# YiyangShao/splendor-gym

Measured on AMD Instinct MI355X. Metric: env-steps/sec (whole node), 2p 65536 tables/GPU, higher is better.
Workload: dtype int32

## Files before the change

### include/splendor_amd.h

```cpp
#ifndef SPLENDOR_AMD_H
#define SPLENDOR_AMD_H

#include <stdint.h>

#include "splendor_table.h"

#ifdef __cplusplus
extern "C" {
#endif

#define SPL_ABI_VERSION 9

#define SPL_F_ILLEGAL 0x01
#define SPL_F_DRAW 0x02
#define SPL_F_TURN_LIMIT 0x04
#define SPL_F_AFTER_TERMINAL 0x08
#define SPL_F_OOB 0x10
#define SPL_F_RESET 0x20
#define SPL_F_RNG_LIMIT 0x40
#define SPL_F_FAULT 0x80

#define SPL_POLICY_UNIFORM 0
#define SPL_POLICY_GREEDY_V1 1
#define SPL_POLICY_BASIC_PRIORITY 2
// ... 26 lines not shown
    int32_t autoreset;
    int32_t policy;
    int32_t *next_actions;
    const uint64_t *ply_base;
    uint64_t policy_seed;
    uint64_t ply;
    int64_t table0;
    float *ep_return;
    uint32_t *ep_count;
    uint8_t *info;
    uint64_t *errors;
    uint8_t *obs_u8;
    const uint8_t *gate_terminated;
    const uint8_t *gate_flags;
} spl_step_args_t;

int spl_abi_version(void);
const char *spl_last_error(void);

int spl_ctx_create(int device, const int32_t *cards, const int32_t *nobles, spl_ctx_t **out);
int spl_ctx_destroy(spl_ctx_t *ctx);
int spl_ctx_set_refill_period(spl_ctx_t *ctx, int period);
int spl_ctx_set_refill_fused(spl_ctx_t *ctx, int fused);
int spl_ctx_set_rollout_pipeline(spl_ctx_t *ctx, int on);
int spl_ctx_set_rollout_delegation(spl_ctx_t *ctx, int every);
int spl_ctx_set_partner_lead(spl_ctx_t *ctx, int lead);
int spl_ctx_set_step_tail(spl_ctx_t *ctx, int mode);
const char *spl_rollout_kernel_name(spl_ctx_t *ctx, int32_t n, int32_t players, int32_t per_step_outputs);

int spl_ctx_faults(spl_ctx_t *ctx, uint64_t *launch, int clear);
const volatile uint64_t *spl_ctx_fault_word(spl_ctx_t *ctx);
uint64_t spl_ctx_launches(spl_ctx_t *ctx);
int spl_host_mapped(const void *host, int32_t *same_address);

int64_t spl_arena_bytes(int32_t n, int32_t players);
int spl_arena_init(spl_ctx_t *ctx, spl_arena_t *arena, void *stream);

int spl_reset(spl_ctx_t *ctx, spl_arena_t *arena, const uint64_t *pcg, const uint8_t *reset_mask,
              int32_t *obs, int8_t *mask, void *stream);

int spl_deal(spl_ctx_t *ctx, spl_arena_t *arena, const uint32_t *engine_seeds, const uint8_t *deal_mask,
             int32_t *obs, int8_t *mask, void *stream);

int spl_step(spl_ctx_t *ctx, spl_arena_t *arena, const spl_step_args_t *args, void *stream);

int spl_rollout(spl_ctx_t *ctx, spl_arena_t *arena, const spl_step_args_t *args, int32_t steps,
                int32_t per_step_outputs, void *stream);

int spl_refill(spl_ctx_t *ctx, spl_arena_t *arena, void *stream);

int spl_encode(spl_ctx_t *ctx, spl_arena_t *arena, int32_t *obs, void *stream);
int spl_legal(spl_ctx_t *ctx, spl_arena_t *arena, int8_t *mask, void *stream);

int spl_sample_uniform(spl_ctx_t *ctx, int32_t n, const int8_t *mask, int32_t *actions,
                       uint64_t seed, uint64_t ply, int64_t table0, void *stream);

int spl_step_info(int32_t n, const uint8_t *flags, uint8_t *info, uint64_t *errors, void *stream);

int spl_table_download(spl_ctx_t *ctx, spl_arena_t *arena, int32_t first, int32_t count,
                       spl_table_t *host, void *stream);
int spl_table_upload(spl_ctx_t *ctx, spl_arena_t *arena, int32_t first, int32_t count,
                     const spl_table_t *host, void *stream);

int spl_debug_set_stream_limit(int outputs);

int spl_debug_set_spin_limit(int64_t polls);
int spl_debug_partner_stats(uint64_t *stats, int clear);

int spl_debug_bounds_flags(uint32_t *flags, int clear);

int64_t spl_ctx_token_lut(spl_ctx_t *ctx, uint32_t *out, int64_t words);

#ifdef __cplusplus
}
#endif
#endif
```

### splendor-gym_amd/csrc/spl_engine.hip

```cpp
#include <hip/hip_runtime.h>
#include <stdint.h>
#include <string.h>

#include <algorithm>
#include <atomic>
#include <map>
#include <mutex>
#include <string>
#include <vector>

#include "../../include/splendor_amd.h"
#include "spl_layout.h"
#include "spl_rng.h"

namespace spl {

struct KArena {
    uint32_t *planes;
    uint32_t *pool;
    uint8_t *slots;
    uint8_t *pcg;
    int n;
    uint8_t *deleg;
    uint32_t *dflags;
// ... 2979 lines not shown
        wave_lds_sync();
        if (obs) store_obs_block(L.rows, rows, obs + (size_t)t0 * kObsDim);
        if (mask_out) store_mask_block(L.mask, L.mbits, rows, mask_out + (size_t)t0 * 45);
    }
    if (valid) store_tab(T, A, t, lm, Tb.mtag);
}

constexpr int kRefillLds = 40 * 1024;
template <int P>
__global__ __launch_bounds__(64) void k_refill(KArena A) {
    __shared__ uint8_t scr_all[kRefillLds] __attribute__((aligned(16)));
    const int t = blockIdx.x * 64 + lane_id();
    if (t >= A.n) return;
    const size_t mi = (size_t)SW_MISC * A.n + t;
    const uint32_t misc = A.planes[mi];
    if (pend_of(misc) == 0) return;
    Deal pool;
    bool pool_dirty = false;
    A.planes[mi] = refill_table<P>(A, t, misc, &scr_all[lane_id() * kScratchStride],
                                   reinterpret_cast<uint32_t *>(&scr_all[64 * kScratchStride]), pool, pool_dirty);
    if (pool_dirty) store_pool(A, t, pool);
}

template <int P>
__global__ __launch_bounds__(64) void k_observe(KArena A, KTables Tb, int32_t *obs, int8_t *mask_out) {
    __shared__ BlockLDS L;
    const int lane = lane_id();
    const int t0 = blockIdx.x * 64;
    const int t = t0 + lane;
    const bool valid = t < A.n;
    const int rows = min(64, A.n - t0);
    load_tables_lds(L, Tb);
    Tab<P> T;
    if (valid) load_tab(T, A, t);
    else fresh_state(T, 0u, empty_deal());
    wave_lds_sync();
    if (obs) encode_row(T, L.rows, L);
    L.mask[lane] = valid ? legal_of(T, L) : 0ull;
    wave_lds_sync();
    if (obs) {
        store_obs_block(L.rows, rows, obs + (size_t)t0 * kObsDim);
        if (__any(valid && get_moves(T.sw) > 255)) {
            __builtin_amdgcn_s_waitcnt(0);
            if (valid && get_moves(T.sw) > 255) obs[(size_t)t * kObsDim + 295] = get_moves(T.sw);
        }
    }
// ... 168 lines not shown
}

using namespace spl;

struct spl_ctx_s {
    int device;
    uint4 *cards;
    uint2 *nobles;
    uint4 *lut;
    int refill_period;
    int refill_fused;
    int pipeline;
    int resident[7][5];
    int deleg_every;
    int partner_lead;
    uint32_t mtag;
    int step_tail;
    int64_t step_tail_blocks;
    uint64_t *fault_host;
    uint64_t *fault_dev;
    uint64_t launches;
    void *stage;
    size_t stage_bytes;
};

static thread_local std::string g_err;

int spl_fail(int code, const std::string &msg) {
    g_err = msg;
    return code;
}
static inline int fail(int code, const std::string &msg) { return spl_fail(code, msg); }

#define HIP_TRY(expr)                                                                   \
    do {                                                                                \
        hipError_t e_ = (expr);                                                         \
        if (e_ != hipSuccess) return fail(SPL_E_HIP, std::string(#expr ": ") + hipGetErrorString(e_)); \
    } while (0)

static KTables ktables(const spl_ctx_t *c) { return KTables{c->cards, c->nobles, c->lut, c->mtag}; }

static int check_arena(const spl_ctx_t *ctx, const spl_arena_t *a) {
    if (!ctx) return fail(SPL_E_ARG, "null context");
    if (!a || !a->base) return fail(SPL_E_ARG, "null arena");
    if (a->players < 2 || a->players > 4) return fail(SPL_E_ARG, "players must be 2..4");
    if (a->n <= 0) return fail(SPL_E_ARG, "arena must hold at least one table");
    if (((uintptr_t)a->base & 255u) != 0) return fail(SPL_E_ARG, "arena base must be 256-byte aligned");
    if (a->bytes < spl_arena_bytes(a->n, a->players)) return fail(SPL_E_ARG, "arena too small");
    return SPL_OK;
}

static KArena karena(const spl_arena_t *a) {
    const ArenaLayout L = arena_layout(a->n, a->players);
    uint8_t *b = static_cast<uint8_t *>(a->base);
    return KArena{reinterpret_cast<uint32_t *>(b + L.planes), reinterpret_cast<uint32_t *>(b + L.pool), b + L.slots,
                  b + L.pcg, a->n, b + L.deleg, reinterpret_cast<uint32_t *>(b + L.dflags),
                  reinterpret_cast<uint32_t *>(b + L.legal)};
}

static int launch_check() {
    hipError_t e = hipGetLastError();
    if (e != hipSuccess) return fail(SPL_E_HIP, std::string("kernel launch: ") + hipGetErrorString(e));
    return SPL_OK;
}

static inline unsigned blocks_for(int64_t n) { return (unsigned)((n + 63) / 64); }

extern "C" {

int spl_abi_version(void) { return SPL_ABI_VERSION; }

// ... 108 lines not shown
        memcpy(&nrec[i], b, 8);
    }
    HIP_TRY(hipSetDevice(device));
    int resident[7][5] = {};
    {
        int cus = 0;
        HIP_TRY(hipDeviceGetAttribute(&cus, hipDeviceAttributeMultiprocessorCount, device));
        for (int shape = 2; shape <= 6; ++shape)
            for (int p = 2; p <= 4; ++p) {
                const RolloutKernel &k = rollout_kernel(shape, true, p);
                int occ = 0;
                HIP_TRY(hipOccupancyMaxActiveBlocksPerMultiprocessor(&occ, k.fn, k.threads, 0));
                resident[shape][p] = occ * cus;
            }
    }
    spl_ctx_t *c = new spl_ctx_t();
    c->device = device;
    c->mtag = card_table_tag(crec, nrec);
    c->refill_period = 64;
    c->refill_fused = 1;
    c->deleg_every = kDelegEveryDefault;
    c->partner_lead = kPartnerLeadDefault;
    c->step_tail = -1;
    {
        int cus = 0;
        HIP_TRY(hipDeviceGetAttribute(&cus, hipDeviceAttributeMultiprocessorCount, device));
        c->step_tail_blocks = 3 * (int64_t)cus;
    }
    c->pipeline = 1;
    memcpy(c->resident, resident, sizeof(resident));
    if (hipMalloc(&c->cards, sizeof(uint4) * 90) != hipSuccess || hipMalloc(&c->nobles, sizeof(uint2) * 10) != hipSuccess ||
        hipMalloc(&c->lut, sizeof(uint4) * kLutEntries) != hipSuccess) {
        spl_ctx_destroy(c);
        return fail(SPL_E_HIP, "hipMalloc of constant tables failed");
    }
    if (hipHostMalloc(reinterpret_cast<void **>(&c->fault_host), sizeof(uint64_t),
                      hipHostMallocMapped | hipHostMallocCoherent) != hipSuccess ||
        hipHostGetDevicePointer(reinterpret_cast<void **>(&c->fault_dev), c->fault_host, 0) != hipSuccess) {
        spl_ctx_destroy(c);
        return fail(SPL_E_HIP, "hipHostMalloc of the fault word failed");
    }
    *c->fault_host = 0;
    HIP_TRY(hipMemcpy(c->cards, crec.data(), sizeof(uint4) * 90, hipMemcpyHostToDevice));
    HIP_TRY(hipMemcpy(c->nobles, nrec.data(), sizeof(uint2) * 10, hipMemcpyHostToDevice));
    hipLaunchKernelGGL(k_build_lut, dim3(blocks_for(kLutEntries)), dim3(64), 0, 0, c->lut);
    if (int r = launch_check()) {
        spl_ctx_destroy(c);
        return r;
    }
    HIP_TRY(hipDeviceSynchronize());
    *out = c;
    return SPL_OK;
}

int spl_ctx_destroy(spl_ctx_t *ctx) {
    if (!ctx) return SPL_OK;
    if (ctx->cards) (void)hipFree(ctx->cards);
    if (ctx->nobles) (void)hipFree(ctx->nobles);
    if (ctx->lut) (void)hipFree(ctx->lut);
    if (ctx->stage) (void)hipFree(ctx->stage);
    if (ctx->fault_host) (void)hipHostFree(ctx->fault_host);
    delete ctx;
    return SPL_OK;
}

int spl_ctx_faults(spl_ctx_t *ctx, uint64_t *launch, int clear) {
    if (!ctx || !launch) return fail(SPL_E_ARG, "null argument");
    volatile uint64_t *w = ctx->fault_host;
    *launch = *w;
    if (clear) *w = 0;
    return SPL_OK;
}

const volatile uint64_t *spl_ctx_fault_word(spl_ctx_t *ctx) {
    if (!ctx) {
        fail(SPL_E_ARG, "null ctx");
        return nullptr;
    }
    return ctx->fault_host;
// ... 35 lines not shown
    return SPL_OK;
}

int spl_debug_partner_stats(uint64_t *stats, int clear) {
    if (!stats) return fail(SPL_E_ARG, "stats must be non-null");
    unsigned long long v[2] = {0ull, 0ull};
    HIP_TRY(hipDeviceSynchronize());
    HIP_TRY(hipMemcpyFromSymbol(v, HIP_SYMBOL(g_partner_stats), sizeof(v)));
    stats[0] = v[0];
    stats[1] = v[1];
    if (clear) {
        const unsigned long long z[2] = {0ull, 0ull};
        HIP_TRY(hipMemcpyToSymbol(HIP_SYMBOL(g_partner_stats), z, sizeof(z)));
    }
    return SPL_OK;
}

int spl_ctx_set_rollout_delegation(spl_ctx_t *ctx, int every) {
    if (!ctx || every < 0 || (every > 0 && every < 4)) return fail(SPL_E_ARG, "delegation period must be 0 or >= 4");
    ctx->deleg_every = every;
    return SPL_OK;
}

int spl_ctx_set_refill_fused(spl_ctx_t *ctx, int fused) {
    if (!ctx) return fail(SPL_E_ARG, "null ctx");
    ctx->refill_fused = fused != 0;
    return SPL_OK;
}

int64_t spl_ctx_token_lut(spl_ctx_t *ctx, uint32_t *out, int64_t words) {
    const int64_t need = (int64_t)kLutEntries * 4;
    if (!ctx) return fail(SPL_E_ARG, "null context");
    if (!out) return need;
    if (words < need) return fail(SPL_E_ARG, "output too small");
    HIP_TRY(hipMemcpy(out, ctx->lut, need * 4, hipMemcpyDeviceToHost));
    return need;
}

#define DISPATCH_P(P_, call)                        \
    switch (P_) {                                   \
        case 2: { constexpr int PP = 2; call; } break; \
        case 3: { constexpr int PP = 3; call; } break; \
        case 4: { constexpr int PP = 4; call; } break; \
        default: return fail(SPL_E_ARG, "players must be 2..4"); \
    }

int spl_reset(spl_ctx_t *ctx, spl_arena_t *arena, const uint64_t *pcg, const uint8_t *reset_mask, int32_t *obs,
              int8_t *mask, void *stream) {
    if (int r = check_arena(ctx, arena)) return r;
    if (obs && ((uintptr_t)obs & 15u)) return fail(SPL_E_ARG, "obs must be 16-byte aligned");
    if (mask && ((uintptr_t)mask & 3u)) return fail(SPL_E_ARG, "mask must be 4-byte aligned");
    const KArena A = karena(arena);
    hipStream_t s = static_cast<hipStream_t>(stream);
    DISPATCH_P(arena->players, hipLaunchKernelGGL(k_reset<PP>, dim3(blocks_for(arena->n)), dim3(64), 0, s, A,
                                                  ktables(ctx), pcg, reset_mask, obs, mask, (const uint32_t *)nullptr));
    if (int r = launch_check()) return r;
    arena->steps = 0;
    return SPL_OK;
}

int spl_deal(spl_ctx_t *ctx, spl_arena_t *arena, const uint32_t *engine_seeds, const uint8_t *deal_mask,
             int32_t *obs, int8_t *mask, void *stream) {
    if (int r = check_arena(ctx, arena)) return r;
    if (!engine_seeds) return fail(SPL_E_ARG, "engine_seeds is required");
    if (obs && ((uintptr_t)obs & 15u)) return fail(SPL_E_ARG, "obs must be 16-byte aligned");
    if (mask && ((uintptr_t)mask & 3u)) return fail(SPL_E_ARG, "mask must be 4-byte aligned");
    const KArena A = karena(arena);
    hipStream_t s = static_cast<hipStream_t>(stream);
    DISPATCH_P(arena->players, hipLaunchKernelGGL(k_reset<PP>, dim3(blocks_for(arena->n)), dim3(64), 0, s, A,
                                                  ktables(ctx), (const uint64_t *)nullptr, deal_mask, obs, mask,
                                                  engine_seeds));
    return launch_check();
}

int spl_arena_init(spl_ctx_t *ctx, spl_arena_t *arena, void *stream) {
    if (int r = check_arena(ctx, arena)) return r;
    hipStream_t s = static_cast<hipStream_t>(stream);
    HIP_TRY(hipMemsetAsync(arena->base, 0, (size_t)spl_arena_bytes(arena->n, arena->players), s));
    const KArena A = karena(arena);
    HIP_TRY(hipMemsetD32Async(reinterpret_cast<hipDeviceptr_t>(A.planes + (size_t)SW_MISC * arena->n),
                              (int)((uint32_t)(kSlotRecords - 1) << ST_PEND_SHIFT),
                              (size_t)arena->n, s));
    arena->steps = 0;
    arena->epoch = 0;
    return SPL_OK;
}

int spl_refill(spl_ctx_t *ctx, spl_arena_t *arena, void *stream) {
    if (int r = check_arena(ctx, arena)) return r;
    const KArena A = karena(arena);
    hipStream_t s = static_cast<hipStream_t>(stream);
    DISPATCH_P(arena->players, hipLaunchKernelGGL(k_refill<PP>, dim3(blocks_for(arena->n)), dim3(64), 0, s, A));
    if (int r = launch_check()) return r;
    arena->epoch += 1;
    return SPL_OK;
}

static int check_step_args(const spl_step_args_t *a) {
    if (!a || !a->actions || !(a->obs || a->obs_u8) || !a->mask || !a->reward || !a->terminated || !a->flags)
        return fail(SPL_E_ARG, "actions/obs/mask/reward/terminated/flags are required");
    if ((uintptr_t)a->obs_u8 & 15u) return fail(SPL_E_ARG, "obs_u8 must be 16-byte aligned");
    if (!a->gate_terminated != !a->gate_flags) return fail(SPL_E_ARG, "gate_terminated and gate_flags go together");
    if (a->autoreset < 0 || a->autoreset > 2) return fail(SPL_E_ARG, "autoreset must be 0, 1 or 2");
    if (a->policy < SPL_POLICY_UNIFORM || a->policy > SPL_POLICY_BASIC_PRIORITY) return fail(SPL_E_ARG, "unknown policy");
    if (((uintptr_t)a->obs & 15u) || (a->final_obs && ((uintptr_t)a->final_obs & 3u)))
        return fail(SPL_E_ARG, "obs must be 16-byte aligned");
    if ((uintptr_t)a->mask & 3u) return fail(SPL_E_ARG, "mask must be 4-byte aligned");
    return SPL_OK;
}

static KStep kstep(spl_ctx_t *ctx, const spl_step_args_t *a) {
    KStep S;
// ... 4 lines not shown
    S.mask = a->mask;
    S.reward = a->reward;
    S.terminated = a->terminated;
    S.flags = a->flags;
    S.winner = a->winner;
    S.final_obs = a->final_obs;
    S.next_actions = a->next_actions;
    S.ep_return = a->ep_return;
    S.ep_count = a->ep_count;
    S.info = a->info;
    S.obs_u8 = a->obs_u8;
    S.gate_terminated = a->gate_terminated;
    S.gate_flags = a->gate_flags;
    S.errors = reinterpret_cast<unsigned long long *>(a->errors);
    S.ply_base = a->ply_base;
    S.policy_seed = a->policy_seed;
    S.ply = a->ply;
    S.table0 = a->table0;
    S.autoreset = a->autoreset;
    S.policy = a->policy;
    return S;
}

int spl_step(spl_ctx_t *ctx, spl_arena_t *arena, const spl_step_args_t *a, void *stream) {
    if (int r = check_arena(ctx, arena)) return r;
    if (int r = check_step_args(a)) return r;
    const KStep S = kstep(ctx, a);
    const KArena A = karena(arena);
    hipStream_t s = static_cast<hipStream_t>(stream);
    const unsigned blocks = blocks_for(arena->n);
    const int shape = ctx->step_tail >= 0 ? ctx->step_tail
                                          : (((int64_t)blocks <= ctx->step_tail_blocks || a->obs == nullptr) ? 1 : 0);
    const StepKernel &k = kStepKernels[shape * 3 + arena->players - 2];
    hipLaunchKernelGGL(k.fn, dim3(blocks), dim3(k.threads), 0, s, A, ktables(ctx), S);
    if (int r = launch_check()) return r;
    arena->steps += 1;
    if (a->autoreset && ctx->refill_period > 0 && arena->steps % ctx->refill_period == 0)
        return spl_refill(ctx, arena, stream);
    return SPL_OK;
}

static bool rollout_fits(const spl_ctx_t *ctx, int shape, int32_t n, int32_t players) {
    const int tpw = rollout_kernel(shape, true, players).tpw;
    return ((int64_t)n + tpw - 1) / tpw <= ctx->resident[shape][players];
}

static int rollout_shape(const spl_ctx_t *ctx, int32_t n, int32_t players) {
    if (ctx->pipeline != 1) return ctx->pipeline;
    if (rollout_fits(ctx, 5, n, players)) return 5;
    if (rollout_fits(ctx, 4, n, players)) return 4;
    if (players == 2 && rollout_fits(ctx, 6, n, players)) return 6;
    return 2;
}

const char *spl_rollout_kernel_name(spl_ctx_t *ctx, int32_t n, int32_t players, int32_t per_step_outputs) {
    static const char *const one_wave[3] = {"k_rollout<2>", "k_rollout<3>", "k_rollout<4>"};
    if (!ctx || n <= 0 || players < 2 || players > 4) {
        fail(SPL_E_ARG, "spl_rollout_kernel_name: bad arguments");
        return nullptr;
    }
    const int shape = rollout_shape(ctx, n, players);
    return shape == 0 ? one_wave[players - 2] : rollout_kernel(shape, per_step_outputs != 0, players).name;
}

int spl_rollout(spl_ctx_t *ctx, spl_arena_t *arena, const spl_step_args_t *a, int32_t steps, int32_t per_step_outputs,
                void *stream) {
    if (int r = check_arena(ctx, arena)) return r;
    if (int r = check_step_args(a)) return r;
    if (!a->obs) return fail(SPL_E_ARG, "spl_rollout writes int32 obs (obs_u8 is spl_step only)");
    if (a->gate_terminated || a->gate_flags) return fail(SPL_E_ARG, "the gate is spl_step only");
    if (steps < 1) return fail(SPL_E_ARG, "spl_rollout: steps must be >= 1");
    if (per_step_outputs && (arena->n & 3))
        return fail(SPL_E_ARG, "spl_rollout: per-step outputs need a table count divisible by 4 (16-byte obs blocks)");
    const KStep S = kstep(ctx, a);
    const KArena A = karena(arena);
    hipStream_t s = static_cast<hipStream_t>(stream);
    const int64_t before = arena->steps;
    const bool due = a->autoreset && ctx->refill_period > 0 &&
                     (before + steps) / ctx->refill_period != before / ctx->refill_period;
    const int fused = (due && ctx->refill_fused)
                          ? (int)std::min<int64_t>(steps, (before + steps) / ctx->refill_period - before / ctx->refill_period)
                          : 0;
    const int shape = rollout_shape(ctx, arena->n, arena->players);
    if (shape == 0) {
        DISPATCH_P(arena->players, hipLaunchKernelGGL(k_rollout<PP>, dim3(blocks_for(arena->n)), dim3(64), 0, s, A,
                                                      ktables(ctx), S, (int)steps, (int)(per_step_outputs != 0), fused));
    } else {
        const RolloutKernel &k = rollout_kernel(shape, per_step_outputs != 0, arena->players);
        int extra = 0;
        if (k.extra != kExtraNone && rollout_fits(ctx, shape, arena->n, arena->players))
            extra = k.extra == kExtraLead ? ctx->partner_lead : ctx->deleg_every;
        hipLaunchKernelGGL(k.fn, dim3((unsigned)((arena->n + k.tpw - 1) / k.tpw)), dim3(k.threads), 0, s, A, ktables(ctx), S,
                           (int)steps, fused, extra);
    }
    if (int r = launch_check()) return r;
    arena->steps += steps;
    if (fused) arena->epoch += fused;
    else if (due) return spl_refill(ctx, arena, stream);
    return SPL_OK;
}

int spl_encode(spl_ctx_t *ctx, spl_arena_t *arena, int32_t *obs, void *stream) {
    if (int r = check_arena(ctx, arena)) return r;
    if (!obs || ((uintptr_t)obs & 15u)) return fail(SPL_E_ARG, "obs must be non-null and 16-byte aligned");
    const KArena A = karena(arena);
    hipStream_t s = static_cast<hipStream_t>(stream);
    DISPATCH_P(arena->players, hipLaunchKernelGGL(k_observe<PP>, dim3(blocks_for(arena->n)), dim3(64), 0, s, A,
                                                  ktables(ctx), obs, (int8_t *)nullptr));
    return launch_check();
}

int spl_legal(spl_ctx_t *ctx, spl_arena_t *arena, int8_t *mask, void *stream) {
    if (int r = check_arena(ctx, arena)) return r;
    if (!mask || ((uintptr_t)mask & 3u)) return fail(SPL_E_ARG, "mask must be non-null and 4-byte aligned");
    const KArena A = karena(arena);
    hipStream_t s = static_cast<hipStream_t>(stream);
    DISPATCH_P(arena->players, hipLaunchKernelGGL(k_observe<PP>, dim3(blocks_for(arena->n)), dim3(64), 0, s, A,
                                                  ktables(ctx), (int32_t *)nullptr, mask));
    return launch_check();
}

int spl_sample_uniform(spl_ctx_t *ctx, int32_t n, const int8_t *mask, int32_t *actions, uint64_t seed, uint64_t ply,
                       int64_t table0, void *stream) {
    if (!ctx || n <= 0 || !mask || !actions) return fail(SPL_E_ARG, "bad sample arguments");
    hipLaunchKernelGGL(k_sample, dim3(blocks_for(n)), dim3(64), 0, static_cast<hipStream_t>(stream), n, mask, actions,
                       seed, ply, table0);
    return launch_check();
}

int spl_step_info(int32_t n, const uint8_t *flags, uint8_t *info, uint64_t *errors, void *stream) {
    if (n <= 0 || !flags || !info || !errors || ((uintptr_t)errors & 7u)) return fail(SPL_E_ARG, "bad step-info arguments");
    hipLaunchKernelGGL(k_step_info, dim3((unsigned)((n + 255) / 256)), dim3(256), 0, static_cast<hipStream_t>(stream), n,
                       flags, info, reinterpret_cast<unsigned long long *>(errors));
    return launch_check();
}

static int ensure_stage(spl_ctx_t *ctx, size_t bytes) {
    if (ctx->stage_bytes >= bytes) return SPL_OK;
    if (ctx->stage) (void)hipFree(ctx->stage);
    ctx->stage = nullptr;
    ctx->stage_bytes = 0;
    HIP_TRY(hipMalloc(&ctx->stage, bytes));
    ctx->stage_bytes = bytes;
    return SPL_OK;
}

int spl_table_download(spl_ctx_t *ctx, spl_arena_t *arena, int32_t first, int32_t count, spl_table_t *host,
                       void *stream) {
    if (int r = check_arena(ctx, arena)) return r;
    if (!host || first < 0 || count <= 0 || first + count > arena->n) return fail(SPL_E_ARG, "bad download range");
    if (int r = ensure_stage(ctx, sizeof(spl_table_t) * (size_t)count)) return r;
    const KArena A = karena(arena);
    hipStream_t s = static_cast<hipStream_t>(stream);
    spl_table_t *st = static_cast<spl_table_t *>(ctx->stage);
    DISPATCH_P(arena->players, hipLaunchKernelGGL(k_download<PP>, dim3(blocks_for(count)), dim3(64), 0, s, A, first, count, st));
    if (int r = launch_check()) return r;
    HIP_TRY(hipMemcpyAsync(host, st, sizeof(spl_table_t) * (size_t)count, hipMemcpyDeviceToHost, s));
    HIP_TRY(hipStreamSynchronize(s));
    return SPL_OK;
}

static int validate_view(const spl_table_t &v, int P) {
    if (v.num_players != P) return fail(SPL_E_RANGE, "num_players does not match the arena");
    for (int c = 0; c < 6; ++c)
        if (v.bank[c] < 0 || v.bank[c] > 255) return fail(SPL_E_RANGE, "bank out of range");
    int owned = 0;
    for (int q = 0; q < P; ++q) {
        const spl_player_t &p = v.players[q];
        for (int c = 0; c < 6; ++c)
            if (p.tokens[c] < 0 || p.tokens[c] > 255) return fail(SPL_E_RANGE, "tokens out of range");
        for (int c = 0; c < 5; ++c)
            if (p.bonuses[c] < 0 || p.bonuses[c] > 255) return fail(SPL_E_RANGE, "bonuses out of range");
// ... 9 lines not shown
    for (int k = 0; k < 12; ++k)
        if (v.board[k] < -1 || v.board[k] >= 90) return fail(SPL_E_RANGE, "board card id out of range");
    for (int t = 0; t < 3; ++t) {
        if (v.deck_len[t] < 0 || v.deck_len[t] > tier_size(t)) return fail(SPL_E_RANGE, "deck too long for its record");
        for (int k = 0; k < v.deck_len[t]; ++k)
            if (v.decks[t][k] < 0 || v.decks[t][k] >= 90) return fail(SPL_E_RANGE, "deck card id out of range");
    }
    if (v.n_nobles < 0 || v.n_nobles > 5) return fail(SPL_E_RANGE, "visible noble slots out of range");
    int taken = 0;
    for (int s = 0; s < v.n_nobles; ++s) {
        if (v.nobles[s] >= 10 || v.nobles[s] < -1) return fail(SPL_E_RANGE, "noble id out of range");
        taken += v.nobles[s] < 0;
    }
    if (owned > taken) return fail(SPL_E_RANGE, "players hold more nobles than taken slots");
    if (v.to_play < 0 || v.to_play >= P) return fail(SPL_E_RANGE, "to_play out of range");
    if (v.turn_count < 0 || v.turn_count > 255) return fail(SPL_E_RANGE, "turn_count out of range");
    if (v.move_count < 0 || v.move_count > 508) return fail(SPL_E_RANGE, "move_count out of range (<= 508)");
    if (v.winner < -1 || v.winner >= P) return fail(SPL_E_RANGE, "winner out of range");
    return SPL_OK;
}

int spl_table_upload(spl_ctx_t *ctx, spl_arena_t *arena, int32_t first, int32_t count, const spl_table_t *host,
                     void *stream) {
    if (int r = check_arena(ctx, arena)) return r;
    if (!host || first < 0 || count <= 0 || first + count > arena->n) return fail(SPL_E_ARG, "bad upload range");
    for (int i = 0; i < count; ++i)
        if (int r = validate_view(host[i], arena->players)) return r;
    if (int r = ensure_stage(ctx, sizeof(spl_table_t) * (size_t)count)) return r;
    const KArena A = karena(arena);
    hipStream_t s = static_cast<hipStream_t>(stream);
    spl_table_t *st = static_cast<spl_table_t *>(ctx->stage);
    HIP_TRY(hipMemcpyAsync(st, host, sizeof(spl_table_t) * (size_t)count, hipMemcpyHostToDevice, s));
    DISPATCH_P(arena->players, hipLaunchKernelGGL(k_upload<PP>, dim3(blocks_for(count)), dim3(64), 0, s, A, first, count, st));
    if (int r = launch_check()) return r;
    HIP_TRY(hipStreamSynchronize(s));
    return SPL_OK;
}

}
```

### splendor-gym_amd/splendor_gym/_native.py

```python
import ctypes
import os

import numpy as np

LIB_NAME = "libsplendor_amd.so"
ABI_VERSION = 9

POLICY_UNIFORM, POLICY_GREEDY_V1, POLICY_BASIC_PRIORITY = 0, 1, 2
F_ILLEGAL, F_DRAW, F_TURN_LIMIT = 0x01, 0x02, 0x04
F_AFTER_TERMINAL, F_OOB, F_RESET, F_RNG_LIMIT = 0x08, 0x10, 0x20, 0x40
F_FAULT = 0x80

OBS_DIM = 297
OBS_U8 = 300
NUM_ACTIONS = 45

c_void_p, c_int32, c_int64, c_uint64 = ctypes.c_void_p, ctypes.c_int32, ctypes.c_int64, ctypes.c_uint64


class ArenaDesc(ctypes.Structure):
    _fields_ = [("base", c_void_p), ("bytes", c_int64), ("n", c_int32), ("players", c_int32),
                ("steps", c_int64), ("epoch", c_int64)]


# ... 34 lines not shown
    _fields_ = [("episode", c_void_p), ("group_of", c_void_p), ("group_prev", c_void_p), ("pool_slots", c_void_p),
                ("pool_len", c_int32), ("p_current", ctypes.c_float), ("seed", c_uint64), ("table0", c_int64)]


DUAL_ILLEGAL, DUAL_DRAW, DUAL_TURN_LIMIT = 0x01, 0x02, 0x04


PLAYER_DTYPE = np.dtype([("tokens", "<i4", 6), ("bonuses", "<i4", 5), ("prestige", "<i4"),
                         ("n_reserved", "<i4"), ("reserved", "<i4", 3), ("revealed", "<i4", 3),
                         ("n_nobles", "<i4"), ("nobles", "<i4", 5)])
TABLE_DTYPE = np.dtype([("num_players", "<i4"), ("bank", "<i4", 6), ("players", PLAYER_DTYPE, 4),
                        ("board", "<i4", 12), ("deck_len", "<i4", 3), ("decks", "<i4", (3, 40)),
                        ("n_nobles", "<i4"), ("nobles", "<i4", 5), ("to_play", "<i4"),
                        ("turn_count", "<i4"), ("move_count", "<i4"), ("game_over", "<i4"),
                        ("winner", "<i4"), ("turn_limit_reached", "<i4")])

SIGNATURES = {
    "spl_abi_version": ([], c_int32),
    "spl_last_error": ([], ctypes.c_char_p),
    "spl_ctx_create": ([c_int32, c_void_p, c_void_p, ctypes.POINTER(c_void_p)], c_int32),
    "spl_ctx_destroy": ([c_void_p], c_int32),
    "spl_ctx_set_refill_period": ([c_void_p, c_int32], c_int32),
    "spl_ctx_set_refill_fused": ([c_void_p, c_int32], c_int32),
    "spl_ctx_set_rollout_pipeline": ([c_void_p, c_int32], c_int32),
    "spl_ctx_set_rollout_delegation": ([c_void_p, c_int32], c_int32),
    "spl_ctx_set_partner_lead": ([c_void_p, c_int32], c_int32),
    "spl_ctx_set_step_tail": ([c_void_p, c_int32], c_int32),
    "spl_ctx_token_lut": ([c_void_p, c_void_p, c_int64], c_int64),
    "spl_ctx_faults": ([c_void_p, ctypes.POINTER(c_uint64), c_int32], c_int32),
    "spl_ctx_fault_word": ([c_void_p], c_void_p),
    "spl_ctx_launches": ([c_void_p], c_uint64),
    "spl_host_mapped": ([c_void_p, ctypes.POINTER(c_int32)], c_int32),
    "spl_debug_set_spin_limit": ([c_int64], c_int32),
    "spl_debug_partner_stats": ([c_void_p, c_int32], c_int32),
    "spl_rollout_kernel_name": ([c_void_p, c_int32, c_int32, c_int32], ctypes.c_char_p),
    "spl_arena_bytes": ([c_int32, c_int32], c_int64),
    "spl_arena_init": ([c_void_p, ctypes.POINTER(ArenaDesc), c_void_p], c_int32),
    "spl_reset": ([c_void_p, ctypes.POINTER(ArenaDesc), c_void_p, c_void_p, c_void_p, c_void_p, c_void_p],
                  c_int32),
    "spl_debug_set_stream_limit": ([c_int32], c_int32),
    "spl_debug_bounds_flags": ([c_void_p, c_int32], c_int32),
    "spl_deal": ([c_void_p, ctypes.POINTER(ArenaDesc), c_void_p, c_void_p, c_void_p, c_void_p, c_void_p], c_int32),
    "spl_step": ([c_void_p, ctypes.POINTER(ArenaDesc), ctypes.POINTER(StepArgs), c_void_p], c_int32),
    "spl_rollout": ([c_void_p, ctypes.POINTER(ArenaDesc), ctypes.POINTER(StepArgs), c_int32, c_int32, c_void_p],
                    c_int32),
    "spl_refill": ([c_void_p, ctypes.POINTER(ArenaDesc), c_void_p], c_int32),
# ... 76 lines not shown
```

### splendor-gym_amd/splendor_gym/device.py

```python
import ctypes

import numpy as np

from . import _native
from ._native import NUM_ACTIONS, OBS_DIM, OBS_U8, TABLE_DTYPE, ArenaDesc, LaunchFault, StepArgs, check, ptr
from .engine.state import load_tables
from .seeding import pcg64_states


class Engine:

    DEFAULT_REFILL = {2: 64, 3: 32, 4: 16}

    def __init__(self, num_tables, num_players=2, device=None, refill_period=None, table0=0, refill_fused=True,
                 pipeline=True, delegation=None, cards=None, partner_lead=None, host_io=False, step_tail=None):
        torch = _native.require_gpu()
        self.torch = torch
        self.lib = _native.load_library()
        if not 2 <= num_players <= 4:
            raise ValueError("num_players must be 2..4")
        if num_tables <= 0:
            raise ValueError("num_tables must be positive")
        self.n, self.P, self.table0 = int(num_tables), int(num_players), int(table0)
        self.device = torch.device(device) if device is not None else torch.device("cuda", torch.cuda.current_device())
        if self.device.index is None:
            self.device = torch.device("cuda", torch.cuda.current_device())
        self._settings = (refill_period, refill_fused, pipeline, delegation, partner_lead)
        self._step_tail = step_tail
        self.ctx = None
        self._fault_carry = 0
        self._create_ctx(cards)
        nbytes = int(self.lib.spl_arena_bytes(self.n, self.P))
        dev = self.device
        self._arena_raw = torch.zeros(nbytes + 256, dtype=torch.uint8, device=dev)
        off = (-self._arena_raw.data_ptr()) % 256
        self.arena = self._arena_raw[off:off + nbytes]
        self.desc = ArenaDesc(self.arena.data_ptr(), nbytes, self.n, self.P, 0, 0)
        self._step_args = {}
        n = self.n
        specs = [("obs", torch.int32, (n, OBS_DIM)), ("mask", torch.int8, (n, NUM_ACTIONS)),
                 ("reward", torch.float32, (n,)), ("terminated", torch.uint8, (n,)), ("flags", torch.uint8, (n,)),
                 ("winner", torch.int8, (n,)), ("actions", torch.int32, (n,)),
                 ("final_obs", torch.int32, (n, OBS_DIM))]
        offs, off = [], 0
        for name, dt, shape in specs:
            nb = int(np.prod(shape)) * torch.empty((), dtype=dt).element_size()
            offs.append((name, dt, shape, off, nb))
            off = (off + nb + 255) // 256 * 256
        self.host_io = bool(host_io)
        self.io = (torch.zeros(off, dtype=torch.uint8, pin_memory=True) if self.host_io
                   else torch.zeros(off, dtype=torch.uint8, device=dev))
# ... 18 lines not shown
        if tbl.shape != (90, 8):
            raise ValueError("card table must be int32 [90, 8]")
        ctx = ctypes.c_void_p()
        with torch.cuda.device(self.device):
            check(self.lib, self.lib.spl_ctx_create(self.device.index, tbl.ctypes.data, nobles.ctypes.data,
                                                    ctypes.byref(ctx)))
        self.ctx = ctx
        self._fault_word = ctypes.c_uint64.from_address(self.lib.spl_ctx_fault_word(ctx))
        self.custom_cards = None if cards is None else tbl.copy()
        refill_period, refill_fused, pipeline, delegation, partner_lead = self._settings
        num_players = self.P
        if refill_period is None:
            refill_period = self.DEFAULT_REFILL.get(int(num_players), 16)
        check(self.lib, self.lib.spl_ctx_set_refill_period(self.ctx, int(refill_period)))
        check(self.lib, self.lib.spl_ctx_set_refill_fused(self.ctx, 1 if refill_fused else 0))
        pipe = {"always": 2, "half": 3, "dealer": 4, "dealer2": 5, "quad": 6}.get(pipeline, 1 if pipeline else 0)
        check(self.lib, self.lib.spl_ctx_set_rollout_pipeline(self.ctx, pipe))
        if delegation is not None:
            check(self.lib, self.lib.spl_ctx_set_rollout_delegation(self.ctx, int(delegation)))
        if partner_lead is not None:
            check(self.lib, self.lib.spl_ctx_set_partner_lead(self.ctx, int(partner_lead)))
        if self._step_tail is not None:
            check(self.lib, self.lib.spl_ctx_set_step_tail(self.ctx, int(self._step_tail)))

    def set_card_table(self, cards=None):
        same = (cards is None and self.custom_cards is None) or (
            cards is not None and self.custom_cards is not None and np.array_equal(cards, self.custom_cards))
        if same:
            return
        self.torch.cuda.synchronize(self.device)
        old = self.ctx
        self._fault_carry = self.faults()
        self._create_ctx(cards)
        self.lib.spl_ctx_destroy(old)

    def faults(self):
        if self._fault_word is None:
            return self._fault_carry
        return self._fault_carry or int(self._fault_word.value)

    def check_faults(self):
        if self.ctx is None:
            raise RuntimeError("splendor engine: used after close()")
        f = self.faults()
        if f:
            raise LaunchFault(f"splendor engine: launch {f} lost an internal hand-off; its outputs from the faulted "
# ... 153 lines not shown
                     flags=bufs["flags"].data_ptr(), winner=ptr(bufs.get("winner")),
                     final_obs=ptr(bufs.get("final_obs")) if final_obs else None, autoreset=1, policy=int(policy),
                     next_actions=None if next_actions is None else next_actions.data_ptr(),
                     ply_base=None if ply_base is None else ply_base.data_ptr(),
                     policy_seed=int(policy_seed) & (2**64 - 1), ply=int(ply) & (2**64 - 1), table0=self.table0,
                     ep_return=None if ep_return is None else ep_return.data_ptr(),
                     ep_count=None if ep_count is None else ep_count.data_ptr())
        with torch.cuda.device(self.device):
            check(self.lib, self.lib.spl_rollout(self.ctx, ctypes.byref(self.desc), ctypes.byref(a), int(steps),
                                                 per_step, self.stream()))
        self._keep_actions = (actions, bufs)
        return bufs

    def rollout_kernel_name(self, per_step=True):
        name = self.lib.spl_rollout_kernel_name(self.ctx, self.n, self.P, 1 if per_step else 0)
        if name is None:
            check(self.lib, -1)
        return name.decode()

    def refill(self):
        with self.torch.cuda.device(self.device):
            check(self.lib, self.lib.spl_refill(self.ctx, ctypes.byref(self.desc), self.stream()))

    def encode(self, out=None):
        out = self.obs if out is None else out
        with self.torch.cuda.device(self.device):
            check(self.lib, self.lib.spl_encode(self.ctx, ctypes.byref(self.desc), ptr(out), self.stream()))
        return out

    def legal(self, out=None):
        out = self.mask if out is None else out
        with self.torch.cuda.device(self.device):
            check(self.lib, self.lib.spl_legal(self.ctx, ctypes.byref(self.desc), ptr(out), self.stream()))
        return out

    def sample_uniform(self, mask=None, out=None, seed=0, ply=0):
        mask = self.mask if mask is None else mask
        out = self.actions if out is None else out
        with self.torch.cuda.device(self.device):
            check(self.lib, self.lib.spl_sample_uniform(self.ctx, self.n, ptr(mask), ptr(out), int(seed), int(ply),
                                                        self.table0, self.stream()))
        return out

    def download(self, first=0, count=None):
        count = self.n - first if count is None else count
        out = np.zeros(count, TABLE_DTYPE)
# ... 18 lines not shown
```

Before: 4.399 billion.

## Stage refill deals on a side stream overlapped with steps before commit

Adds a side stream that runs a k_refill_stage kernel a few steps before each refill. It precomputes each table's next deal, keyed by a snapshot of the table's PCG state. At the refill point a commit kernel copies the staged record into the slot and advances the RNG when the snapshot still matches, and falls back to the full refill otherwise. The aim is to hide the costly deal generation behind step kernels. In exchange it adds extra memory, event syncs, atomic stat counters, and may add contention with the concurrent step kernels.

```diff
diff --git a/include/splendor_amd.h b/include/splendor_amd.h
--- a/include/splendor_amd.h
+++ b/include/splendor_amd.h
@@ -72,6 +72,7 @@
 int spl_ctx_destroy(spl_ctx_t *ctx);
 int spl_ctx_set_refill_period(spl_ctx_t *ctx, int period);
 int spl_ctx_set_refill_fused(spl_ctx_t *ctx, int fused);
+int spl_ctx_set_refill_overlap(spl_ctx_t *ctx, int on);
 int spl_ctx_set_rollout_pipeline(spl_ctx_t *ctx, int on);
 int spl_ctx_set_rollout_delegation(spl_ctx_t *ctx, int every);
 int spl_ctx_set_partner_lead(spl_ctx_t *ctx, int lead);
@@ -116,6 +117,7 @@
 
 int spl_debug_set_spin_limit(int64_t polls);
 int spl_debug_partner_stats(uint64_t *stats, int clear);
+int spl_debug_refill_stats(uint64_t *stats, int clear);
 
 int spl_debug_bounds_flags(uint32_t *flags, int clear);
 
diff --git a/splendor-gym_amd/csrc/spl_engine.hip b/splendor-gym_amd/csrc/spl_engine.hip
--- a/splendor-gym_amd/csrc/spl_engine.hip
+++ b/splendor-gym_amd/csrc/spl_engine.hip
@@ -3025,6 +3025,106 @@
     if (pool_dirty) store_pool(A, t, pool);
 }
 
+constexpr int kStageBytes = 192;
+constexpr int kStageValid = 116 / 4;
+constexpr int kStageSnap = 128, kStageAdv = 168;
+constexpr int kStageLds = 64 * kScratchStride + 624 * 4;
+constexpr int kStageScr = 100;
+constexpr int kStageMtWords = 624;
+
+constexpr int kStatWays = 256;
+__device__ unsigned long long g_refill_stats[3][kStatWays];
+
+__device__ __forceinline__ void count_lanes(unsigned long long *counter, bool mine) {
+    const uint64_t active = __ballot(1), hits = __ballot(mine);
+    if (hits && lane_id() == __ffsll((unsigned long long)active) - 1)
+        atomicAdd(counter + blockIdx.x % kStatWays, (unsigned long long)__popcll(hits));
+}
+
+__device__ __forceinline__ bool stage_matches(const uint8_t *e, const Pcg64 &g) {
+    const uint64_t *p = reinterpret_cast<const uint64_t *>(e + kStageSnap);
+    const uint32_t *q = reinterpret_cast<const uint32_t *>(p + 4);
+    return reinterpret_cast<const uint32_t *>(e)[kStageValid] != 0u && p[0] == g.s_hi && p[1] == g.s_lo &&
+           p[2] == g.inc_hi && p[3] == g.inc_lo && q[0] == g.has32 && q[1] == g.u32;
+}
+
+template <int P>
+__global__ __launch_bounds__(64) void k_refill_stage(KArena A, uint8_t *stage, uint32_t *mtx_all) {
+    __shared__ uint8_t scr_all[64 * kStageScr] __attribute__((aligned(16)));
+    const int t = blockIdx.x * 64 + lane_id();
+    if (t >= A.n) return;
+    uint8_t *e = stage + (size_t)t * kStageBytes;
+    Pcg64 g = load_pcg(A, t);
+    if (stage_matches(e, g)) return;
+    uint32_t *ew = reinterpret_cast<uint32_t *>(e);
+    ew[kStageValid] = 0u;
+    uint64_t *p = reinterpret_cast<uint64_t *>(e + kStageSnap);
+    uint32_t *q = reinterpret_cast<uint32_t *>(p + 4);
+    p[0] = g.s_hi;
+    p[1] = g.s_lo;
+    p[2] = g.inc_hi;
+    p[3] = g.inc_lo;
+    q[0] = g.has32;
+    q[1] = g.u32;
+    const uint32_t seed = g.valid() ? g.engine_seed() : 0u;
+    Deal d;
+    deal_into(seed, P, e, &scr_all[lane_id() * kStageScr], d, mtx_all + (size_t)blockIdx.x * kStageMtWords);
+    uint64_t *a = reinterpret_cast<uint64_t *>(e + kStageAdv);
+    a[0] = g.s_hi;
+    a[1] = g.s_lo;
+    reinterpret_cast<uint32_t *>(a + 2)[0] = g.has32;
+    reinterpret_cast<uint32_t *>(a + 2)[1] = g.u32;
+    ew[kStageValid] = 1u;
+    count_lanes(g_refill_stats[0], true);
+}
+
+template <int P>
+__global__ __launch_bounds__(64) void k_refill_commit(KArena A, uint8_t *stage) {
+    __shared__ uint8_t scr_all[kStageLds] __attribute__((aligned(16)));
+    const int t = blockIdx.x * 64 + lane_id();
+    if (t >= A.n) return;
+    const size_t mi = (size_t)SW_MISC * A.n + t;
+    uint8_t *e = stage + (size_t)t * kStageBytes;
+    uint32_t *ew = reinterpret_cast<uint32_t *>(e);
+    const uint32_t misc = A.planes[mi];
+    const int pend = pend_of(misc);
+    if (pend == 0) return;
+    Pcg64 g = load_pcg(A, t);
+    const bool staged = ew[kStageValid] != 0u, hit = stage_matches(e, g);
+    count_lanes(g_refill_stats[1], hit);
+    count_lanes(g_refill_stats[2], staged && !hit);
+    Deal pool;
+    bool pool_dirty = false;
+    if (hit) {
+        const int slot = (active_of(misc) + kSlotRecords - pend) % kSlotRecords;
+        const uint4 *eq = reinterpret_cast<const uint4 *>(e);
+        uint4 *rq = reinterpret_cast<uint4 *>(slot_rec(A, t, slot));
+        const uint4 r6 = eq[6], r7 = eq[7];
+#pragma unroll
+        for (int k = 0; k < 6; ++k) rq[k] = eq[k];
+        rq[6] = r6;
+        rq[7] = uint4{r7.x, 0u, 0u, r7.w};
+        if (g.valid()) {
+            const uint64_t *a = reinterpret_cast<const uint64_t *>(e + kStageAdv);
+            g.s_hi = a[0];
+            g.s_lo = a[1];
+            g.has32 = reinterpret_cast<const uint32_t *>(a + 2)[0];
+            g.u32 = reinterpret_cast<const uint32_t *>(a + 2)[1];
+            store_pcg(A, t, g);
+        }
+        ew[kStageValid] = 0u;
+        if (pend == kSlotRecords - 1) {
+            pool = Deal{{r6.x, r6.y, r6.z}, r6.w, r7.x};
+            pool_dirty = true;
+        }
+        A.planes[mi] = (misc & ~ST_PEND) | ((uint32_t)(pend - 1) << ST_PEND_SHIFT);
+    } else {
+        A.planes[mi] = refill_table<P>(A, t, misc, &scr_all[lane_id() * kScratchStride],
+                                       reinterpret_cast<uint32_t *>(&scr_all[64 * kScratchStride]), pool, pool_dirty);
+    }
+    if (pool_dirty) store_pool(A, t, pool);
+}
+
 template <int P>
 __global__ __launch_bounds__(64) void k_observe(KArena A, KTables Tb, int32_t *obs, int8_t *mask_out) {
     __shared__ BlockLDS L;
@@ -3239,6 +3339,13 @@
     uint64_t launches;
     void *stage;
     size_t stage_bytes;
+    int refill_overlap;
+    hipStream_t side;
+    hipEvent_t ev_fork, ev_staged;
+    uint8_t *deals;
+    size_t deals_bytes;
+    const void *deals_for;
+    const void *staging;
 };
 
 static thread_local std::string g_err;
@@ -3264,6 +3371,41 @@
     if (a->n <= 0) return fail(SPL_E_ARG, "arena must hold at least one table");
     if (((uintptr_t)a->base & 255u) != 0) return fail(SPL_E_ARG, "arena base must be 256-byte aligned");
     if (a->bytes < spl_arena_bytes(a->n, a->players)) return fail(SPL_E_ARG, "arena too small");
+    return SPL_OK;
+}
+
+constexpr int kRefillLead = 8;
+
+static int settle_refill(spl_ctx_t *ctx, hipStream_t s) {
+    if (!ctx->staging) return SPL_OK;
+    ctx->staging = nullptr;
+    HIP_TRY(hipStreamWaitEvent(s, ctx->ev_staged, 0));
+    return SPL_OK;
+}
+#define CHECK_SETTLED(ctx_, arena_, stream_)                                            \
+    do {                                                                                \
+        if (int r_ = check_arena(ctx_, arena_)) return r_;                              \
+        if (int r_ = settle_refill(ctx_, static_cast<hipStream_t>(stream_))) return r_; \
+    } while (0)
+
+static inline size_t deals_bytes_for(int64_t n) {
+    return (size_t)n * kStageBytes + (size_t)((n + 63) / 64) * kStageMtWords * 4;
+}
+
+static int ensure_deals(spl_ctx_t *ctx, const spl_arena_t *arena, hipStream_t s) {
+    const size_t need = deals_bytes_for(arena->n);
+    if (ctx->deals_bytes < need) {
+        if (ctx->deals) (void)hipFree(ctx->deals);
+        ctx->deals = nullptr;
+        ctx->deals_bytes = 0;
+        ctx->deals_for = nullptr;
+        HIP_TRY(hipMalloc(reinterpret_cast<void **>(&ctx->deals), need));
+        ctx->deals_bytes = need;
+    }
+    if (ctx->deals_for != arena->base) {
+        HIP_TRY(hipMemsetAsync(ctx->deals, 0, need, s));
+        ctx->deals_for = arena->base;
+    }
     return SPL_OK;
 }
 
@@ -3418,6 +3560,7 @@
     c->deleg_every = kDelegEveryDefault;
     c->partner_lead = kPartnerLeadDefault;
     c->step_tail = -1;
+    c->refill_overlap = 1;
     {
         int cus = 0;
         HIP_TRY(hipDeviceGetAttribute(&cus, hipDeviceAttributeMultiprocessorCount, device));
@@ -3437,6 +3580,12 @@
         return fail(SPL_E_HIP, "hipHostMalloc of the fault word failed");
     }
     *c->fault_host = 0;
+    if (hipStreamCreateWithFlags(&c->side, hipStreamNonBlocking) != hipSuccess ||
+        hipEventCreateWithFlags(&c->ev_fork, hipEventDisableTiming) != hipSuccess ||
+        hipEventCreateWithFlags(&c->ev_staged, hipEventDisableTiming) != hipSuccess) {
+        spl_ctx_destroy(c);
+        return fail(SPL_E_HIP, "creating the refill stream failed");
+    }
     HIP_TRY(hipMemcpy(c->cards, crec.data(), sizeof(uint4) * 90, hipMemcpyHostToDevice));
     HIP_TRY(hipMemcpy(c->nobles, nrec.data(), sizeof(uint2) * 10, hipMemcpyHostToDevice));
     hipLaunchKernelGGL(k_build_lut, dim3(blocks_for(kLutEntries)), dim3(64), 0, 0, c->lut);
@@ -3451,6 +3600,13 @@
 
 int spl_ctx_destroy(spl_ctx_t *ctx) {
     if (!ctx) return SPL_OK;
+    if (ctx->side) {
+        (void)hipStreamSynchronize(ctx->side);
+        (void)hipStreamDestroy(ctx->side);
+    }
+    if (ctx->ev_fork) (void)hipEventDestroy(ctx->ev_fork);
+    if (ctx->ev_staged) (void)hipEventDestroy(ctx->ev_staged);
+    if (ctx->deals) (void)hipFree(ctx->deals);
     if (ctx->cards) (void)hipFree(ctx->cards);
     if (ctx->nobles) (void)hipFree(ctx->nobles);
     if (ctx->lut) (void)hipFree(ctx->lut);
@@ -3532,6 +3688,28 @@
     return SPL_OK;
 }
 
+int spl_ctx_set_refill_overlap(spl_ctx_t *ctx, int on) {
+    if (!ctx) return fail(SPL_E_ARG, "null ctx");
+    ctx->refill_overlap = on != 0;
+    return SPL_OK;
+}
+
+int spl_debug_refill_stats(uint64_t *stats, int clear) {
+    if (!stats) return fail(SPL_E_ARG, "stats must be non-null");
+    static unsigned long long v[3][kStatWays];
+    HIP_TRY(hipDeviceSynchronize());
+    HIP_TRY(hipMemcpyFromSymbol(v, HIP_SYMBOL(g_refill_stats), sizeof(v)));
+    for (int i = 0; i < 3; ++i) {
+        stats[i] = 0;
+        for (int w = 0; w < kStatWays; ++w) stats[i] += v[i][w];
+    }
+    if (clear) {
+        memset(v, 0, sizeof(v));
+        HIP_TRY(hipMemcpyToSymbol(HIP_SYMBOL(g_refill_stats), v, sizeof(v)));
+    }
+    return SPL_OK;
+}
+
 int spl_ctx_set_refill_fused(spl_ctx_t *ctx, int fused) {
     if (!ctx) return fail(SPL_E_ARG, "null ctx");
     ctx->refill_fused = fused != 0;
@@ -3557,7 +3735,7 @@
 
 int spl_reset(spl_ctx_t *ctx, spl_arena_t *arena, const uint64_t *pcg, const uint8_t *reset_mask, int32_t *obs,
               int8_t *mask, void *stream) {
-    if (int r = check_arena(ctx, arena)) return r;
+    CHECK_SETTLED(ctx, arena, stream);
     if (obs && ((uintptr_t)obs & 15u)) return fail(SPL_E_ARG, "obs must be 16-byte aligned");
     if (mask && ((uintptr_t)mask & 3u)) return fail(SPL_E_ARG, "mask must be 4-byte aligned");
     const KArena A = karena(arena);
@@ -3571,7 +3749,7 @@
 
 int spl_deal(spl_ctx_t *ctx, spl_arena_t *arena, const uint32_t *engine_seeds, const uint8_t *deal_mask,
              int32_t *obs, int8_t *mask, void *stream) {
-    if (int r = check_arena(ctx, arena)) return r;
+    CHECK_SETTLED(ctx, arena, stream);
     if (!engine_seeds) return fail(SPL_E_ARG, "engine_seeds is required");
     if (obs && ((uintptr_t)obs & 15u)) return fail(SPL_E_ARG, "obs must be 16-byte aligned");
     if (mask && ((uintptr_t)mask & 3u)) return fail(SPL_E_ARG, "mask must be 4-byte aligned");
@@ -3584,7 +3762,7 @@
 }
 
 int spl_arena_init(spl_ctx_t *ctx, spl_arena_t *arena, void *stream) {
-    if (int r = check_arena(ctx, arena)) return r;
+    CHECK_SETTLED(ctx, arena, stream);
     hipStream_t s = static_cast<hipStream_t>(stream);
     HIP_TRY(hipMemsetAsync(arena->base, 0, (size_t)spl_arena_bytes(arena->n, arena->players), s));
     const KArena A = karena(arena);
@@ -3593,11 +3771,15 @@
                               (size_t)arena->n, s));
     arena->steps = 0;
     arena->epoch = 0;
+    if (ctx->refill_overlap) {
+        ctx->deals_for = nullptr;
+        if (int r = ensure_deals(ctx, arena, s)) return r;
+    }
     return SPL_OK;
 }
 
 int spl_refill(spl_ctx_t *ctx, spl_arena_t *arena, void *stream) {
-    if (int r = check_arena(ctx, arena)) return r;
+    CHECK_SETTLED(ctx, arena, stream);
     const KArena A = karena(arena);
     hipStream_t s = static_cast<hipStream_t>(stream);
     DISPATCH_P(arena->players, hipLaunchKernelGGL(k_refill<PP>, dim3(blocks_for(arena->n)), dim3(64), 0, s, A));
@@ -3648,12 +3830,54 @@
     return S;
 }
 
+static int fork_point(spl_ctx_t *ctx, spl_arena_t *arena, hipStream_t s, bool *forked) {
+    *forked = false;
+    if (ctx->deals_bytes < deals_bytes_for(arena->n) || ctx->deals_for != arena->base) {
+        hipStreamCaptureStatus cap = hipStreamCaptureStatusNone;
+        HIP_TRY(hipStreamIsCapturing(s, &cap));
+        if (cap != hipStreamCaptureStatusNone) return SPL_OK;
+        if (int r = ensure_deals(ctx, arena, s)) return r;
+    }
+    HIP_TRY(hipEventRecord(ctx->ev_fork, s));
+    *forked = true;
+    return SPL_OK;
+}
+
+static int stage_refill(spl_ctx_t *ctx, spl_arena_t *arena) {
+    const KArena A = karena(arena);
+    HIP_TRY(hipStreamWaitEvent(ctx->side, ctx->ev_fork, 0));
+    DISPATCH_P(arena->players, hipLaunchKernelGGL(k_refill_stage<PP>, dim3(blocks_for(arena->n)), dim3(64), 0, ctx->side,
+                                                  A, ctx->deals,
+                                                  reinterpret_cast<uint32_t *>(ctx->deals + (size_t)arena->n * kStageBytes)));
+    if (int r = launch_check()) return r;
+    HIP_TRY(hipEventRecord(ctx->ev_staged, ctx->side));
+    ctx->staging = arena->base;
+    return SPL_OK;
+}
+
+static int commit_refill(spl_ctx_t *ctx, spl_arena_t *arena, hipStream_t s) {
+    ctx->staging = nullptr;
+    HIP_TRY(hipStreamWaitEvent(s, ctx->ev_staged, 0));
+    const KArena A = karena(arena);
+    DISPATCH_P(arena->players, hipLaunchKernelGGL(k_refill_commit<PP>, dim3(blocks_for(arena->n)), dim3(64), 0, s, A,
+                                                  ctx->deals));
+    if (int r = launch_check()) return r;
+    arena->epoch += 1;
+    return SPL_OK;
+}
+
 int spl_step(spl_ctx_t *ctx, spl_arena_t *arena, const spl_step_args_t *a, void *stream) {
     if (int r = check_arena(ctx, arena)) return r;
     if (int r = check_step_args(a)) return r;
+    if (ctx->staging && (ctx->staging != arena->base || a->autoreset != 1 || a->gate_flags))
+        if (int r = settle_refill(ctx, static_cast<hipStream_t>(stream))) return r;
     const KStep S = kstep(ctx, a);
     const KArena A = karena(arena);
     hipStream_t s = static_cast<hipStream_t>(stream);
+    bool forked = false;
+    if (ctx->refill_overlap && a->autoreset == 1 && !a->gate_flags && !ctx->staging &&
+        ctx->refill_period > kRefillLead && arena->steps % ctx->refill_period == ctx->refill_period - kRefillLead)
+        if (int r = fork_point(ctx, arena, s, &forked)) return r;
     const unsigned blocks = blocks_for(arena->n);
     const int shape = ctx->step_tail >= 0 ? ctx->step_tail
                                           : (((int64_t)blocks <= ctx->step_tail_blocks || a->obs == nullptr) ? 1 : 0);
@@ -3661,8 +3885,10 @@
     hipLaunchKernelGGL(k.fn, dim3(blocks), dim3(k.threads), 0, s, A, ktables(ctx), S);
     if (int r = launch_check()) return r;
     arena->steps += 1;
+    if (forked)
+        if (int r = stage_refill(ctx, arena)) return r;
     if (a->autoreset && ctx->refill_period > 0 && arena->steps % ctx->refill_period == 0)
-        return spl_refill(ctx, arena, stream);
+        return ctx->staging ? commit_refill(ctx, arena, s) : spl_refill(ctx, arena, stream);
     return SPL_OK;
 }
 
@@ -3691,7 +3917,7 @@
 
 int spl_rollout(spl_ctx_t *ctx, spl_arena_t *arena, const spl_step_args_t *a, int32_t steps, int32_t per_step_outputs,
                 void *stream) {
-    if (int r = check_arena(ctx, arena)) return r;
+    CHECK_SETTLED(ctx, arena, stream);
     if (int r = check_step_args(a)) return r;
     if (!a->obs) return fail(SPL_E_ARG, "spl_rollout writes int32 obs (obs_u8 is spl_step only)");
     if (a->gate_terminated || a->gate_flags) return fail(SPL_E_ARG, "the gate is spl_step only");
@@ -3727,7 +3953,7 @@
 }
 
 int spl_encode(spl_ctx_t *ctx, spl_arena_t *arena, int32_t *obs, void *stream) {
-    if (int r = check_arena(ctx, arena)) return r;
+    CHECK_SETTLED(ctx, arena, stream);
     if (!obs || ((uintptr_t)obs & 15u)) return fail(SPL_E_ARG, "obs must be non-null and 16-byte aligned");
     const KArena A = karena(arena);
     hipStream_t s = static_cast<hipStream_t>(stream);
@@ -3737,7 +3963,7 @@
 }
 
 int spl_legal(spl_ctx_t *ctx, spl_arena_t *arena, int8_t *mask, void *stream) {
-    if (int r = check_arena(ctx, arena)) return r;
+    CHECK_SETTLED(ctx, arena, stream);
     if (!mask || ((uintptr_t)mask & 3u)) return fail(SPL_E_ARG, "mask must be non-null and 4-byte aligned");
     const KArena A = karena(arena);
     hipStream_t s = static_cast<hipStream_t>(stream);
@@ -3773,7 +3999,7 @@
 
 int spl_table_download(spl_ctx_t *ctx, spl_arena_t *arena, int32_t first, int32_t count, spl_table_t *host,
                        void *stream) {
-    if (int r = check_arena(ctx, arena)) return r;
+    CHECK_SETTLED(ctx, arena, stream);
     if (!host || first < 0 || count <= 0 || first + count > arena->n) return fail(SPL_E_ARG, "bad download range");
     if (int r = ensure_stage(ctx, sizeof(spl_table_t) * (size_t)count)) return r;
     const KArena A = karena(arena);
@@ -3829,7 +4055,7 @@
 
 int spl_table_upload(spl_ctx_t *ctx, spl_arena_t *arena, int32_t first, int32_t count, const spl_table_t *host,
                      void *stream) {
-    if (int r = check_arena(ctx, arena)) return r;
+    CHECK_SETTLED(ctx, arena, stream);
     if (!host || first < 0 || count <= 0 || first + count > arena->n) return fail(SPL_E_ARG, "bad upload range");
     for (int i = 0; i < count; ++i)
         if (int r = validate_view(host[i], arena->players)) return r;
diff --git a/splendor-gym_amd/splendor_gym/_native.py b/splendor-gym_amd/splendor_gym/_native.py
--- a/splendor-gym_amd/splendor_gym/_native.py
+++ b/splendor-gym_amd/splendor_gym/_native.py
@@ -80,6 +80,8 @@
     "spl_ctx_destroy": ([c_void_p], c_int32),
     "spl_ctx_set_refill_period": ([c_void_p, c_int32], c_int32),
     "spl_ctx_set_refill_fused": ([c_void_p, c_int32], c_int32),
+    "spl_ctx_set_refill_overlap": ([c_void_p, c_int32], c_int32),
+    "spl_debug_refill_stats": ([c_void_p, c_int32], c_int32),
     "spl_ctx_set_rollout_pipeline": ([c_void_p, c_int32], c_int32),
     "spl_ctx_set_rollout_delegation": ([c_void_p, c_int32], c_int32),
     "spl_ctx_set_partner_lead": ([c_void_p, c_int32], c_int32),
diff --git a/splendor-gym_amd/splendor_gym/device.py b/splendor-gym_amd/splendor_gym/device.py
--- a/splendor-gym_amd/splendor_gym/device.py
+++ b/splendor-gym_amd/splendor_gym/device.py
@@ -13,7 +13,8 @@
     DEFAULT_REFILL = {2: 64, 3: 32, 4: 16}
 
     def __init__(self, num_tables, num_players=2, device=None, refill_period=None, table0=0, refill_fused=True,
-                 pipeline=True, delegation=None, cards=None, partner_lead=None, host_io=False, step_tail=None):
+                 pipeline=True, delegation=None, cards=None, partner_lead=None, host_io=False, step_tail=None,
+                 refill_overlap=None):
         torch = _native.require_gpu()
         self.torch = torch
         self.lib = _native.load_library()
@@ -27,6 +28,7 @@
             self.device = torch.device("cuda", torch.cuda.current_device())
         self._settings = (refill_period, refill_fused, pipeline, delegation, partner_lead)
         self._step_tail = step_tail
+        self._refill_overlap = refill_overlap
         self.ctx = None
         self._fault_carry = 0
         self._create_ctx(cards)
@@ -91,6 +93,8 @@
             check(self.lib, self.lib.spl_ctx_set_partner_lead(self.ctx, int(partner_lead)))
         if self._step_tail is not None:
             check(self.lib, self.lib.spl_ctx_set_step_tail(self.ctx, int(self._step_tail)))
+        if self._refill_overlap is not None:
+            check(self.lib, self.lib.spl_ctx_set_refill_overlap(self.ctx, 1 if self._refill_overlap else 0))
 
     def set_card_table(self, cards=None):
         same = (cards is None and self.custom_cards is None) or (
@@ -290,6 +294,18 @@
         with self.torch.cuda.device(self.device):
             check(self.lib, self.lib.spl_refill(self.ctx, ctypes.byref(self.desc), self.stream()))
 
+    def refill_stats(self, clear=False):
+        v = (ctypes.c_uint64 * 3)()
+        with self.torch.cuda.device(self.device):
+            check(self.lib, self.lib.spl_debug_refill_stats(v, 1 if clear else 0))
+        return tuple(int(x) for x in v)
+
+    def pcg_records(self):
+        n, off = self.n, 0
+        for nbytes in ((9 + 4 * self.P) * 4 * n, 5 * 4 * n, 4 * 128 * n):
+            off = (off + nbytes + 255) // 256 * 256
+        return self.arena[off:off + 64 * n].view(n, 64)
+
     def encode(self, out=None):
         out = self.obs if out is None else out
         with self.torch.cuda.device(self.device):
```

Measured after the change: 4.376 billion. About the same (-0.5%).
